# BluemlJ/oc_cleanrl

Measured on AMD Instinct MI355X. Metric: env steps/sec (SPS) + PPO updates/sec, ALE/Pong-v5 obj-mode, 1/2/4/8 MI355X, higher is better.
Workload: dtype fp32

## Files before the change

### include/ocppo.h

```cpp
#ifndef OCPPO_H
#define OCPPO_H

#include <stddef.h>
#include <stdint.h>

#ifdef __cplusplus
extern "C" {
#endif

#define OCPPO_ABI_VERSION 30

#define OCPPO_OK 0
#define OCPPO_E_INVALID 1
#define OCPPO_E_LAUNCH 2
#define OCPPO_E_WORKSPACE 3

#define OCPPO_F32 0
#define OCPPO_BF16 1
#define OCPPO_U8 2

#define OCPPO_NET_CHANNELS_LAST 1
#define OCPPO_NET_SCALE_255 2

#define OCPPO_STAT_LOSS 0
#define OCPPO_STAT_PG_LOSS 1
#define OCPPO_STAT_V_LOSS 2
#define OCPPO_STAT_ENTROPY 3
#define OCPPO_STAT_OLD_APPROX_KL 4
#define OCPPO_STAT_APPROX_KL 5
#define OCPPO_STAT_CLIPFRAC 6
#define OCPPO_STAT_ADV_MEAN 7
#define OCPPO_STAT_ADV_STD 8
#define OCPPO_NUM_STATS 9

typedef void* ocppo_stream_t;
typedef struct ocppo_deferred_finish {
  uint64_t opaque[64];
} ocppo_deferred_finish_t;

#if defined(__GNUC__) || defined(__clang__)
#define OCPPO_API __attribute__((visibility("default")))
#else
#define OCPPO_API
// ... 361 lines not shown
                                    int norm_adv, int clip_vloss, float* gp, float* db_h,
                                    float* dwa, float* dwc, float* dba, float* dbc, float* stats,
                                    float* dlogits, float* dvalue, void* workspace,
                                    size_t workspace_bytes, ocppo_deferred_finish_t* finish);
OCPPO_API int ocppo_sum_splits_finish(ocppo_stream_t stream, const float* part, int64_t S,
                                      int64_t n, float* out, const ocppo_deferred_finish_t* finish);
OCPPO_API int ocppo_deferred_finish_run(ocppo_stream_t stream,
                                        const ocppo_deferred_finish_t* finish);

OCPPO_API int ocppo_linear_cache_shift(ocppo_stream_t stream, const float* x, int64_t ldx,
                                       const float* w, const float* b, float* enc,
                                       const float* done, int64_t M, int64_t N, int64_t K,
                                       int64_t W, int relu);
OCPPO_API int ocppo_linear_cache_ring(ocppo_stream_t stream, const float* x, int64_t ldx,
                                      const float* w, const float* b, float* enc,
                                      const float* done, int64_t M, int64_t N, int64_t K,
                                      int64_t W, int64_t slot, int relu);
OCPPO_API int ocppo_linear_act_ring(ocppo_stream_t stream, const float* x, int64_t ldx,
                                    const float* w, const float* b, float* y, int64_t ldy,
                                    int64_t M, int64_t N, int64_t K, int64_t seg, int64_t rot,
                                    int relu);
OCPPO_API int ocppo_conv2d_act(ocppo_stream_t stream, const float* x, int64_t B, int64_t H,
                               int64_t W, int64_t Cin, const float* w, const float* b,
                               int64_t Cout, int64_t KH, int64_t KW, int64_t stride, float* y,
                               int relu);
OCPPO_API int ocppo_store_linear2(ocppo_stream_t stream, const float* frame, const float* reward,
                                  const float* done, int64_t N, int64_t W, int64_t D,
                                  const void* prev_obs, void* obs_out, int obs_dtype,
                                  float* net_obs, float* reward_out, float* done_out, int vecnorm,
                                  double gamma, double epsilon, double clip_reward,
                                  double* ret_state, double* rms_state, const float* w1,
                                  const float* b1, const float* w2, const float* b2, float* y,
                                  int64_t ldy, int64_t N1, int64_t N2);

OCPPO_API int ocppo_cartpole_step(ocppo_stream_t stream, uint64_t seed, const int64_t* actions,
                                  int64_t N, double* state, int64_t* counters, float* obs_out,
                                  float* reward_out, float* done_out, float* ep_state);

#ifdef __cplusplus
}
#endif
#endif
```

### oc_cleanrl_amd/_lib.py

```python
from __future__ import annotations

import ctypes
import os
import re
from pathlib import Path

import torch

PKG = Path(__file__).resolve().parent
LIB_PATH = Path(os.environ.get("OCPPO_LIB", PKG / "lib" / "libocppo_hip.so"))
HEADER = PKG.parent / "include" / "ocppo.h"

OCPPO_ABI_VERSION = 30
OCPPO_OK, OCPPO_E_INVALID, OCPPO_E_LAUNCH, OCPPO_E_WORKSPACE = 0, 1, 2, 3
OCPPO_F32, OCPPO_BF16, OCPPO_U8 = 0, 1, 2
OCPPO_X6_MBITS_ROWS = 2
STAT_NAMES = ("loss", "pg_loss", "v_loss", "entropy", "old_approx_kl", "approx_kl", "clipfrac",
              "adv_mean", "adv_std")
OCPPO_NUM_STATS = len(STAT_NAMES)

P, I64, U64, D, I, SZ = (ctypes.c_void_p, ctypes.c_int64, ctypes.c_uint64, ctypes.c_double,
                         ctypes.c_int, ctypes.c_size_t)

SIGNATURES: dict[str, tuple[type, list]] = {
    "ocppo_abi_version": (I, []),
    "ocppo_last_error": (ctypes.c_char_p, []),
    "ocppo_gae": (I, [P, P, P, P, P, P, I64, I64, D, D, P, P]),
    "ocppo_minibatch_adv_stats": (I, [P, P, P, I64, I64, P]),
    "ocppo_minibatch_prepare": (I, [P, P, I64, I64, P, P, P, P, P, P, P, P, P, P, P]),
    "ocppo_ppo_loss_workspace_bytes": (SZ, [I64, I64]),
    "ocppo_ppo_loss_fwd_bwd": (I, [P, P, P, I64, I64, P, P, P, P, P, P, P, D, D, D, I, I, P, P, P,
                                   P, SZ]),
    "ocppo_clip_adam_workspace_bytes": (SZ, [I64]),
    "ocppo_clip_adam_step": (I, [P, P, P, P, P, I64, P, D, D, D, D, D, P, P, SZ, I, P, P, P, P,
                                 P]),
    "ocppo_categorical_sample": (I, [P, P, P, P, I64, I64, I64, I64, P, P, P, P, P]),
    "ocppo_policy_head_sample": (I, [P, P, I64, I64, P, P, P, P, P, P, I64, I64, I64, P, P, P, P,
                                     P]),
    "ocppo_torch_exponential_geometry": (I, [I64, I64, I64, P, P]),
    "ocppo_philox_exponential": (I, [P, P, I64, P, I64, I64]),
    "ocppo_philox_exponential_steps": (I, [P, P, I64, I64, P, I64, I64, I64]),
    "ocppo_categorical_logprob_entropy": (I, [P, P, P, I64, I64, P, P]),
    "ocppo_categorical_logprob_entropy_bwd": (I, [P, P, P, P, P, I64, I64, P]),
    "ocppo_rollout_store": (I, [P, P, I, P, P, I64, I64, I64, P, P, I, P, P, P, I, P]),
    "ocppo_obs_reset": (I, [P, P, I, I64, I64, I64, P, I, P, I]),
    "ocppo_gather_rows": (I, [P, P, I, P, I64, I64, P]),
# ... 51 lines not shown
    "ocppo_sum_splits_finish": (I, [P, P, I64, I64, P, P]),
    "ocppo_sum_splits_act": (I, [P, P, I64, I64, I64, P, I, P]),
    "ocppo_gemm_x6_gather": (I, [P, P, I64, I64, P, I64, I64, P, I64, I64, I64, I64, I64, I64, P,
                                 I, P, P, I64, I64, I]),
    "ocppo_frames_expand_index": (I, [P, P, P, I64, P, I64, I64, I64, P]),
    "ocppo_gemm_x6_wgrad": (I, [P, P, I64, I64, P, I64, I64, I64, I64, I64, P, I64, P, I64, I64,
                                P, P, P, I64, I, P]),
    "ocppo_conv_x6": (I, [P, I, P, P, P, I64, P, I64, I64, I64, I64, I64, P, I, P, I, P, P, P,
                          P, P, P]),
    "ocppo_conv_x6_u8": (I, [P, I, P, P, I64, I64, I64, I64, I64, I64, P, I64, P, I64, I64, I64,
                             I64, P, I, ctypes.c_float, I, P, P, P, P]),
    "ocppo_deferred_finish_run": (I, [P, P]),
    "ocppo_linear_cache_shift": (I, [P, P, I64, P, P, P, P, I64, I64, I64, I64, I]),
    "ocppo_linear_cache_ring": (I, [P, P, I64, P, P, P, P, I64, I64, I64, I64, I64, I]),
    "ocppo_linear_act_ring": (I, [P, P, I64, P, P, P, I64, I64, I64, I64, I64, I64, I]),
    "ocppo_conv2d_act": (I, [P, P, I64, I64, I64, I64, P, P, I64, I64, I64, I64, P, I]),
    "ocppo_frames_scatter_chunks": (I64, [I64]),
    "ocppo_frames_gather_linear": (I, [P, P, I, I64, I64, I64, I64, P, I64, P, P, I64, I, P, P, P,
                                       P, I64, P, P]),
    "ocppo_q_head_epsilon_greedy": (I, [P, P, I64, I64, P, P, I64, U64, P, I64, D, D, D, P, P, P]),
    "ocppo_dqn_act_step": (I, [P, P, I64, I64, P, P, I64, U64, P, I64, D, D, D, P, P, U64, P, I64,
                               I64, P, P, P, P, I64, P, P, I, P, P, P, I, D, D, D, P, P, P, I64, P,
                               P, P, P, I64]),
    "ocppo_frames_scatter_relu": (I, [P, P, I64, I64, P, I64, P, I64, P, I64, I64, I64, P, P, P,
                                      P]),
    "ocppo_gemm_x6": (I, [P, P, I64, I64, P, I64, I64, P, I64, I64, I64, I64, I64, I64, P, I, P,
                          I64, P, P, P, I, I, P, I64, I64, P, SZ]),
    "ocppo_gemm_x6_sk_workspace_bytes": (SZ, [I]),
    "ocppo_split_planes": (I, [P, I, P, P, P, P, P, P]),
    "ocppo_gae_records": (I, [P, P, P, P, P, P, I64, I64, D, D, P, P, P, P, P]),
    "ocppo_minibatch_prepare_records": (I, [P, P, I64, I64, P, P, P, P, P, P, P]),
    "ocppo_store_linear2": (I, [P, P, P, P, I64, I64, I64, P, P, I, P, P, P, I, D, D, D, P, P, P,
                                P, P, P, P, I64, I64, I64]),
}


class OcppoError(RuntimeError):
    """A C-ABI call returned a non-zero status."""


def header_functions() -> list[str]:
    text = HEADER.read_text()
    return sorted(set(re.findall(r"^\s*(?:const\s+)?[\w\s\*]*?\b(ocppo_\w+)\s*\(", text, re.M)))


def _load() -> ctypes.CDLL:
    if not LIB_PATH.exists():
        raise ImportError(
            f"{LIB_PATH} is missing: the HIP extension is required (no CPU fallback). "
            "Build it with `python -m oc_cleanrl_amd.build`.")
    lib = ctypes.CDLL(str(LIB_PATH))
    for name, (restype, argtypes) in SIGNATURES.items():
        fn = getattr(lib, name)
        fn.restype = restype
        fn.argtypes = argtypes
    ver = lib.ocppo_abi_version()
    if ver != OCPPO_ABI_VERSION:
        raise ImportError(f"{LIB_PATH}: ABI version {ver}, expected {OCPPO_ABI_VERSION}; rebuild")
    return lib


LIB = _load()


def call(name: str, *args) -> None:
    rc = getattr(LIB, name)(*args)
# ... 4 lines not shown
```

### oc_cleanrl_amd/csrc/ocppo_linear.hip

```cpp
#include "ocppo_common.h"

namespace ocppo {

typedef float floatx4 __attribute__((ext_vector_type(4)));

#ifndef OCPPO_LIN_MAX_WAVES
#define OCPPO_LIN_MAX_WAVES 8
#endif
#ifndef OCPPO_LIN_WAVE_TARGET
#define OCPPO_LIN_WAVE_TARGET 4096
#endif
constexpr int kLinMaxWaves = OCPPO_LIN_MAX_WAVES;

template <int CH, bool VEC>
__device__ __forceinline__ void linear_wave_chunks(const float* xr, const float* wr, bool rok,
                                                   bool cok, int K, int g, int c0, int c1,
                                                   floatx4& acc0, floatx4& acc1) {
  for (int cb = c0; cb < c1; cb += CH) {
    float4 a[CH], bb[CH];
#pragma unroll
    for (int q = 0; q < CH; ++q) {
      const int k = (cb + q) * 16 + 4 * g;
      const bool live = cb + q < c1;
      if (VEC && k + 3 < K) {
// ... 498 lines not shown
                                       const float* w, const float* b, float* enc,
                                       const float* done, int64_t M, int64_t N, int64_t K,
                                       int64_t W, int64_t slot, int relu) {
  OCPPO_REQUIRE(M >= 0 && N >= 1 && K >= 1 && W >= 1 && W <= 64 && M <= INT32_MAX &&
                    N <= INT32_MAX && K <= INT32_MAX && slot >= 0 && slot < W,
                "ocppo_linear_cache_ring: bad sizes M=%lld N=%lld K=%lld W=%lld slot=%lld",
                (long long)M, (long long)N, (long long)K, (long long)W, (long long)slot);
  OCPPO_REQUIRE(ldx >= K, "ocppo_linear_cache_ring: ldx=%lld < K", (long long)ldx);
  if (M == 0) return OCPPO_OK;
  OCPPO_REQUIRE(x && w && enc, "ocppo_linear_cache_ring: null pointer");
  OCPPO_REQUIRE((M + 15) / 16 * ((N + 15) / 16) <= INT32_MAX / 8,
                "ocppo_linear_cache_ring: too large");
  const bool vec = K % 4 == 0 && ldx % 4 == 0 && reinterpret_cast<uintptr_t>(x) % 16 == 0 &&
                   reinterpret_cast<uintptr_t>(w) % 16 == 0;
  const CacheOut c{enc, done, static_cast<int>(W), static_cast<int>(slot)};
  clear_stale_error();
  hipStream_t s = as_stream(stream);
  if (relu)
    launch_linear<true, true>(s, vec, x, ldx, w, b, nullptr, 0, (int)M, (int)N, (int)K, c);
  else
    launch_linear<false, true>(s, vec, x, ldx, w, b, nullptr, 0, (int)M, (int)N, (int)K, c);
  return check_launch("ocppo_linear_cache_ring");
}

namespace ocppo {

constexpr int kLin2MaxK1 = 64;
constexpr int kLin2MaxN1 = 512;

template <int S, bool RELU1, bool RELU2, int XDT>
__device__ __forceinline__ void linear2_tile(
    int b, float* smem, const float* __restrict__ x, int64_t ldx, const float* __restrict__ w1,
    const float* __restrict__ b1, const float* __restrict__ w2, const float* __restrict__ b2,
    float* __restrict__ y, int64_t ldy, int M, int N1, int N2, int K1, int ntm, int tiles) {
  const int ldh = N1 + 4;
  float* h1 = smem;
  floatx4* red = reinterpret_cast<floatx4*>(smem + 16 * ldh);
  const int per_xcd = (tiles + 7) / 8;
  const int t = (b % 8) * per_xcd + b / 8;
  if (t >= tiles) return;
  const int tm = t % ntm, tn = t / ntm;
  const int lane = threadIdx.x & 63, wv = threadIdx.x >> 6;
  const int g = lane >> 4, c16 = lane & 15;
  const int row = tm * 16 + c16;
  const bool rok = row < M;
  const float* xr = x + static_cast<int64_t>(rok ? row : 0) * ldx;

  const int nkc = (K1 + 15) / 16;
  const int nct = N1 / 16;
  const int col2 = tn * 16 + c16;
  const bool cok = col2 < N2;
  const float* w2r = w2 + static_cast<int64_t>(cok ? col2 : 0) * N1;
  const int cpw = (nct + S - 1) / S;
  const int c0 = wv * cpw;
  const int c1 = c0 + cpw < nct ? c0 + cpw : nct;
  constexpr int kMaxT = kLin2MaxN1 / 16 / S;
  float4 a1[kLin2MaxK1 / 16];
#pragma unroll
  for (int kc = 0; kc < kLin2MaxK1 / 16; ++kc) {
    const int k = kc * 16 + 4 * g;
    a1[kc].x = (kc < nkc && rok && k + 0 < K1) ? Elem<XDT>::roundtrip(xr[k + 0]) : 0.f;
    a1[kc].y = (kc < nkc && rok && k + 1 < K1) ? Elem<XDT>::roundtrip(xr[k + 1]) : 0.f;
    a1[kc].z = (kc < nkc && rok && k + 2 < K1) ? Elem<XDT>::roundtrip(xr[k + 2]) : 0.f;
    a1[kc].w = (kc < nkc && rok && k + 3 < K1) ? Elem<XDT>::roundtrip(xr[k + 3]) : 0.f;
  }
  float4 b2v[kMaxT];
#pragma unroll
  for (int q = 0; q < kMaxT; ++q) {
    const int c = c0 + q;
    b2v[q] = (c < c1 && cok) ? *reinterpret_cast<const float4*>(w2r + c * 16 + 4 * g)
                             : make_float4(0.f, 0.f, 0.f, 0.f);
  }
#pragma unroll
  for (int q = 0; q < kMaxT; ++q) {
    const int ct = wv + q * S;
    if (ct < nct) {
      const int col = ct * 16 + c16;
      const float* wr = w1 + static_cast<int64_t>(col) * K1;
      floatx4 acc = {0.f, 0.f, 0.f, 0.f};
// ... 185 lines not shown
                "ocppo_store_linear2: bad sizes N=%lld W=%lld D=%lld N1=%lld N2=%lld (D <= 64, "
                "N1 %% 16 == 0, N1 <= 512)", (long long)N, (long long)W, (long long)D,
                (long long)N1, (long long)N2);
  OCPPO_REQUIRE(obs_dtype == OCPPO_F32 || obs_dtype == OCPPO_BF16,
                "ocppo_store_linear2: obs dtype must be OCPPO_F32 or OCPPO_BF16 (object vectors)");
  OCPPO_REQUIRE(frame && reward && done && prev_obs && obs_out && w1 && w2 && y,
                "ocppo_store_linear2: null pointer");
  OCPPO_REQUIRE(prev_obs != obs_out, "ocppo_store_linear2: prev_obs must not alias obs_out");
  OCPPO_REQUIRE(!vecnorm || (ret_state && rms_state && reward_out && reward_out != reward),
                "ocppo_store_linear2: VecNormalize needs ret/rms state and a separate reward_out");
  OCPPO_REQUIRE(reinterpret_cast<uintptr_t>(w2) % 16 == 0,
                "ocppo_store_linear2: w2 must be 16-B aligned");
  StoreLin2Args a;
  a.frame = frame; a.reward = reward; a.done = done; a.N = N; a.D = D; a.W = (int)W;
  a.prev = prev_obs; a.out = obs_out; a.net = net_obs; a.reward_out = reward_out;
  a.done_out = done_out; a.gamma = gamma; a.eps = epsilon; a.clip = clip_reward;
  a.ret = ret_state; a.rms = rms_state;
  a.w1 = w1; a.b1 = b1; a.w2 = w2; a.b2 = b2; a.y = y; a.ldy = ldy;
  a.N1 = (int)N1; a.N2 = (int)N2;
  a.ntm = (int)((N + 15) / 16);
  a.tiles = a.ntm * (int)((N2 + 15) / 16);
  a.lin_blocks = 8 * ((a.tiles + 7) / 8);
  clear_stale_error();
  hipStream_t s = as_stream(stream);
  if (obs_dtype == OCPPO_BF16) {
    if (vecnorm) launch_store_linear2<OCPPO_BF16, true>(s, a);
    else launch_store_linear2<OCPPO_BF16, false>(s, a);
  } else {
    if (vecnorm) launch_store_linear2<OCPPO_F32, true>(s, a);
    else launch_store_linear2<OCPPO_F32, false>(s, a);
  }
  return check_launch("ocppo_store_linear2");
}
```

### oc_cleanrl_amd/csrc/ocppo_synth_env.h

```cpp
#pragma once
#include "ocppo_common.h"

namespace ocppo {

__device__ __forceinline__ uint64_t splitmix64(uint64_t x) {
  x += 0x9E3779B97F4A7C15ull;
  x = (x ^ (x >> 30)) * 0xBF58476D1CE4E5B9ull;
  x = (x ^ (x >> 27)) * 0x94D049BB133111EBull;
  return x ^ (x >> 31);
}
__device__ __forceinline__ float unit24(uint64_t h) {
  return static_cast<float>(h >> 40) * (1.0f / 16777216.0f);
}

__device__ __forceinline__ uint64_t synth_env_key(uint64_t seed, uint64_t step, int64_t n) {
  return splitmix64(splitmix64(splitmix64(seed) + step) + static_cast<uint64_t>(n));
}

__device__ __forceinline__ uint32_t synth_env_obj_base(uint64_t key, int64_t k) {
  const uint64_t h = splitmix64(key + static_cast<uint64_t>(k));
  const int field = static_cast<int>(k & 3);
  if (field == 0) return static_cast<uint32_t>(h % 160u);
  if (field == 1) return static_cast<uint32_t>(h % 210u);
  return static_cast<uint32_t>(1u + h % 16u);
}
__device__ __forceinline__ float synth_env_obj_act(uint32_t base, int64_t k, int64_t a) {
  const uint64_t v = (k == 1) ? (base + 7u * static_cast<uint64_t>(a)) % 210u : base;
  return static_cast<float>(v);
}
__device__ __forceinline__ float synth_env_obj(uint64_t key, int64_t k, int64_t a) {
  return synth_env_obj_act(synth_env_obj_base(key, k), k, a);
}

__device__ __forceinline__ uint8_t synth_env_pixel(uint64_t key, int64_t k, int64_t a) {
  const uint64_t h = splitmix64(key + static_cast<uint64_t>(k));
  uint32_t v = (h % 10u == 0u) ? static_cast<uint32_t>((h >> 8) & 0xFFu) : 0u;
  if (k < 84) v = static_cast<uint32_t>((a * 37) & 0xFF);
  return static_cast<uint8_t>(v);
}

__device__ __forceinline__ void synth_env_outcome(uint64_t key, int64_t n,
                                                  float* __restrict__ reward_out,
                                                  float* __restrict__ done_out,
                                                  float* __restrict__ ep) {
  const float ur = unit24(splitmix64(key ^ 0x5DEECE66Dull));
  const float r = ur < 0.005f ? 1.f : (ur < 0.01f ? -1.f : 0.f);
  const float ud = unit24(splitmix64(key ^ 0xB5297A4Dull));
  const float d = ud < (1.0f / 3500.0f) ? 1.f : 0.f;
  reward_out[n] = r;
  done_out[n] = d;
  if (ep) {
    float* e = ep + n * 5;
    const float run_ret = e[0] + r, run_len = e[1] + 1.f;
    if (d != 0.f) {
      e[2] += run_ret;
      e[3] += run_len;
      e[4] += 1.f;
      e[0] = 0.f;
      e[1] = 0.f;
    } else {
      e[0] = run_ret;
      e[1] = run_len;
    }
  }
}

}
```

### oc_cleanrl_amd/ops.py

```python
from __future__ import annotations

import ctypes

import torch

from . import _lib
from ._lib import OCPPO_BF16, OCPPO_F32, OCPPO_U8, STAT_NAMES, call

_DTYPE_CODE = {torch.float32: OCPPO_F32, torch.bfloat16: OCPPO_BF16, torch.uint8: OCPPO_U8}


def _check(t: torch.Tensor, name: str, dtype: torch.dtype | None = None, device=None,
           numel: int | None = None) -> int:
    if not isinstance(t, torch.Tensor):
        raise TypeError(f"{name}: expected a tensor, got {type(t).__name__}")
    if t.device.type != "cuda":
        raise ValueError(f"{name}: HIP kernels need a GPU tensor, got device {t.device}")
    if device is not None and t.device != device:
        raise ValueError(f"{name}: on {t.device}, expected {device}")
    if dtype is not None and t.dtype != dtype:
        raise ValueError(f"{name}: dtype {t.dtype}, expected {dtype}")
    if not t.is_contiguous():
        raise ValueError(f"{name}: must be contiguous")
    if numel is not None and t.numel() != numel:
# ... 1062 lines not shown


def store_linear2(frame, reward, done, prev_obs, obs_out, net_obs, done_out, reward_out, w1, b1,
                  w2, b2, y, vecnorm_state=None, gamma=0.99, epsilon=1e-8, clip_reward=10.0):
    N, D = frame.shape
    W = obs_out.shape[1]
    dev = frame.device
    f = torch.float32
    if frame.dtype != f:
        raise ValueError("store_linear2: object frames only (f32)")
    if prev_obs.shape != obs_out.shape or prev_obs.dtype != obs_out.dtype or \
            tuple(obs_out.shape) != (N, W, D) or obs_out.dtype not in (torch.float32, torch.bfloat16):
        raise ValueError(f"obs slots must be [N, W, D] f32|bf16, got {tuple(obs_out.shape)} "
                         f"{obs_out.dtype}")
    N1, N2 = w1.shape[0], w2.shape[0]
    if tuple(w1.shape) != (N1, D) or tuple(w2.shape) != (N2, N1) or y.shape[0] != N or \
            y.shape[1] != N2 or y.stride(1) != 1 or y.dtype != f:
        raise ValueError(f"shapes: frame {tuple(frame.shape)}, w1 {tuple(w1.shape)}, "
                         f"w2 {tuple(w2.shape)}, y {tuple(y.shape)}")
    vn = vecnorm_state is not None
    ret, rms = vecnorm_state if vn else (None, None)
    call("ocppo_store_linear2", _stream(dev), _check(frame, "frame", f, dev),
         _check(reward, "reward", f, dev, N), _check(done, "done", f, dev, N), N, W, D,
         _check(prev_obs, "prev_obs", None, dev), _check(obs_out, "obs_out", None, dev),
         _DTYPE_CODE[obs_out.dtype], _opt(net_obs, "net_obs", f, dev, N * W * D),
         _check(reward_out, "reward_out", f, dev, N), _opt(done_out, "done_out", f, dev, N),
         int(vn), float(gamma), float(epsilon), float(clip_reward),
         _opt(ret, "ret_state", torch.float64, dev, N), _opt(rms, "rms_state", torch.float64, dev, 3),
         _check(w1, "w1", f, dev), _opt(b1, "b1", f, dev, N1), _check(w2, "w2", f, dev),
         _opt(b2, "b2", f, dev, N2), y.data_ptr(), y.stride(0) if N > 1 else N2, N1, N2)
    return y


_RB_WS: dict = {}


def _relu_bias_ws(R: int, N: int, dev):
    key = (dev, R, N)
    ws = _RB_WS.get(key)
    if ws is None:
        nb = int(_lib.LIB.ocppo_relu_bias_grad_workspace_bytes(R, N))
        ws = _RB_WS[key] = torch.zeros(nb, dtype=torch.uint8, device=dev)
    return ws


def relu_bias_grad_ok(g) -> bool:
    return (g.is_cuda and g.dtype == torch.float32 and g.dim() == 2 and g.shape[1] % 4 == 0
            and 4 <= g.shape[1] <= 16384 and g.is_contiguous() and g.data_ptr() % 16 == 0)


def relu_bias_grad(g, out=None, db=None, gp=None, bits=None):
    if g.dim() != 2:
        raise ValueError(f"g must be [R, N], got {tuple(g.shape)}")
    R, N = g.shape
    dev = g.device
    f = torch.float32
    if db is None:
        db = torch.empty(N, dtype=f, device=dev)
    if bits is not None:
        gp = torch.empty_like(g) if gp is None else gp
        ws = _relu_bias_ws(R, N, dev)
        call("ocppo_relu_bias_grad_bits", _stream(dev), _check(g, "g", f, dev),
             _check(bits, "bits", torch.int32, dev, R * N // 32), _check(gp, "gp", f, dev, R * N),
             _check(db, "db", f, dev, N), R, N, ws.data_ptr(), ws.numel())
        return gp, db
    if out is not None and gp is None:
# ... 1158 lines not shown
```

### oc_cleanrl_amd/trainer.py

```python
from __future__ import annotations

import json
import math
import os
import time
from dataclasses import asdict
from pathlib import Path

import numpy as np
import torch
import torch.distributed as dist
import torch.nn as nn

from . import agents, frames, gemm_table, ops, rccl
from .rccl import RcclComm, RcclExchange
from .agents import NormalizeImg, PPObj, fused_trunk, linear_relu, make_agent
from .args import Args
from .envs import HostVecEnv, make_device_env


def storage_dtype(args: Args, pixels: bool, integer_obs: bool = True) -> torch.dtype:
    choice = args.obs_storage
    if choice == "auto":
        if pixels:
            return torch.uint8
        return torch.bfloat16 if args.noise_std == 0.0 and integer_obs else torch.float32
    return {"f32": torch.float32, "bf16": torch.bfloat16, "u8": torch.uint8}[choice]


FUSED_HEAD_ENV = True
ADAM_WRITES_PLANES = False
FUSED_HEADS_LOSS_ANY_TRUNK = True
STAGE_ON_SIDE_STREAM = False
U8_ROLLOUT_CONV = True


class FlatGrads:

    def __init__(self, params):
        self.params = [p for p in params if p.requires_grad]
        offs, n = ops.flat_offsets(self.params)
        dev = self.params[0].device
        self.buf = torch.zeros(n, dtype=torch.float32, device=dev)
        for p, off in zip(self.params, offs):
            p.grad = self.buf[off:off + p.numel()].as_strided(p.shape, p.stride())
        self.numel = n

    def zero(self):
        self.buf.zero_()

    def allreduce_mean(self, group=None):
        ws = dist.get_world_size(group)
        dist.all_reduce(self.buf, op=dist.ReduceOp.SUM, group=group)
        self.buf.div_(ws)


class GradExchange:

    def __init__(self, buf, tail_off: int, world: int, scale_in_optimizer: bool, group=None):
        self.buf, self.tail_off, self.world = buf, tail_off, world
        self.scale_in_optimizer, self.group = scale_in_optimizer, group

    def _finish(self):
# ... 190 lines not shown
            self.lr = self.optimizer.lr
        else:
            grads = FlatGrads(self.agent.parameters())
            self.params = grads.params
            self.grad_buf = grads.buf
            self.lr = torch.tensor(a.learning_rate, dtype=torch.float32, device=self.dev)
            self.optimizer = torch.optim.Adam(self.params, lr=self.lr, eps=1e-5, fused=True,
                                              capturable=True)

        T, N = self.T, self.N
        f32 = torch.float32
        dev = self.dev
        self.obs_dtype = storage_dtype(a, self.pixels, not self.host_env and
                                       getattr(self.env, "integer_obs", False))
        self.obs = torch.zeros((T + 1, N) + self.obs_shape, dtype=self.obs_dtype, device=dev)
        self.net_obs = torch.empty((N,) + self.obs_shape, dtype=f32, device=dev,
                                   memory_format=self.net_format).zero_()
        self.actions = torch.zeros((T, N), dtype=torch.int64, device=dev)
        self.logprobs = torch.zeros((T, N), dtype=f32, device=dev)
        self.rewards = torch.zeros((T, N), dtype=f32, device=dev)
        self.dones = torch.zeros((T + 1, N), dtype=f32, device=dev)
        self.values = torch.zeros((T + 1, N), dtype=f32, device=dev)
        self.advantages = torch.zeros((T, N), dtype=f32, device=dev)
        self.returns = torch.zeros((T, N), dtype=f32, device=dev)
        self.noise = torch.zeros((T, N, self.A), dtype=f32, device=dev)
        self.exp_stream = (ops.TorchExpStream(N * self.A, dev)
                           if a.sampling_noise in ("kernel", "head") else None)
        self.enc_cache = (torch.zeros((N, self.obs_shape[0], self.agent.encoding_dim), dtype=f32,
                                      device=dev) if self.frame_cache else None)
        self.rollout_fusion = self.frame_cache and a.rollout_fusion and self._fusable_encoder()
        self.enc_pair = (torch.zeros((N, self.agent.network[2].out_features), dtype=f32, device=dev)
                         if self.rollout_fusion else None)
        self.cache_ring = self.rollout_fusion and a.rollout_cache_ring and self._ring_decoder()
        self.ret_state = torch.zeros(N, dtype=torch.float64, device=dev)
        self.rms_state = torch.tensor([0.0, 1.0, 1e-4], dtype=torch.float64, device=dev)

        self.B = a.local_batch_size
        self.M = a.local_minibatch_size
        self.E = a.update_epochs
        self.nmb = a.num_minibatches
        self.b_inds = np.arange(self.B)
        self.perm_host = torch.empty(self.E * self.B, dtype=torch.int64, pin_memory=True)
        self.perm_dev = torch.zeros(self.E * self.B, dtype=torch.int64, device=dev)
        self.perm_stage = torch.zeros_like(self.perm_dev)
        self.staged = False
        self.staged_rng_state = self.current_rng_state = None
        self.executed_mb = self.E * self.nmb
        self._pending_metrics, self._metrics_host, self._metrics_turn = None, [None, None], 0
        self.perm_event = torch.cuda.Event()
        self.perm_event.record()
        self.copy_stream = (torch.cuda.Stream(dev) if STAGE_ON_SIDE_STREAM and
                            torch.device(dev).type == "cuda" else None)
        self.stage_read = torch.cuda.Event()
        W = self.obs_shape[0]
        self.frame_dedup = (a.update_frame_dedup and isinstance(self.agent, PPObj) and
                            not self.reset_stacks and
                            not self.pixels and len(self.obs_shape) == 2 and
                            len(a.encoder_dims) > 0 and 1 <= W <= 16)
        self.planner = (frames.FramePlanner(T, N, W, a.local_minibatch_size, a.update_epochs,
                                            a.num_minibatches) if self.frame_dedup else None)
        self.plan_host = self.plan_stage = self.plan_dev = self.plan = None
        self.split, self.tail_off, self.cuts = 0, 0, {}
        if self.dp and a.dp_overlap and self.frame_dedup and len(a.encoder_dims) >= 2:
            self.split = 2 * (len(a.encoder_dims) - 1)
            first_tail = self.agent.network[self.split].weight
            offs, _ = ops.flat_offsets(self.params)
# ... 125 lines not shown
        if not self.cache_ring:
            return self.enc_cache
        return torch.roll(self.enc_cache, -(t % self.enc_cache.shape[1]), dims=1)

    def _reset_env(self):
        frame = self.env.frame if self.host_env else self.env.reset()
        if self.reset_stacks:
            ones = torch.ones(self.N, dtype=torch.float32, device=self.dev)
            ops.rollout_store(frame, ones, ones, self.obs[0], self.obs[self.T], self._store_net,
                              scale255=self.prescale, reset_prev=self.env.reset_prev)
        else:
            ops.obs_reset(frame, self.obs[self.T], self._store_net, scale255=self.prescale)
        self.dones[self.T].zero_()

    def _policy_hidden(self, t: int):
        if not self.frame_cache:
            if self.u8_rollout:
                return self.agent.trunk_frames(self.obs[t], self.env_rows)
            return self.agent.trunk(self.net_obs, self.prescale)
        self._policy_encode(t)
        return self._decode_cache(t)

    def _policy_encode(self, t: int):
        ag = self.agent
        if t == 0:
            self.enc_cache.copy_(ag.encode(self.net_obs))
        elif self.rollout_fusion:
            self._store_encode(t)
        else:
            fresh = ag.encode(self.net_obs[:, -1])
            self.timer.bracket("frame_cache", lambda: ops.frame_cache_shift(
                self.enc_cache, fresh, self.dones[t]))

    def _store_encode(self, t: int):
        a, env, net = self.args, self.env, self.agent.network
        lins = [m for m in net[:self.agent._flat] if isinstance(m, nn.Linear)]
        vn = (self.ret_state, self.rms_state) if a.vecnorm_reward else None
        self.timer.bracket("store_encode", lambda: ops.store_linear2(
            env.frame, env.reward, env.done, self.obs[t - 1], self.obs[t], self.net_obs,
            self.dones[t], self.rewards[t - 1], lins[0].weight, lins[0].bias, lins[1].weight,
            lins[1].bias, self.enc_pair, vecnorm_state=vn))
        x = self.enc_pair
        for i, lin in enumerate(lins[2:-1]):
            x = self.timer.bracket("encoder_mid" if i == 0 else f"encoder_mid{i}",
                                   lambda x=x, lin=lin: linear_relu(x, lin))
        last = lins[-1]
        if self.cache_ring:
            W = self.enc_cache.shape[1]
            self.timer.bracket("cache_linear", lambda: ops.linear_cache_ring(
                x, last.weight, last.bias, self.enc_cache, (t - 1) % W, self.dones[t]))
        else:
            self.timer.bracket("cache_linear", lambda: ops.linear_cache_shift(
                x, last.weight, last.bias, self.enc_cache, self.dones[t]))

    def _rollout_step(self, t: int):
        if not self._act(t, env_step=True):
            self.timer.bracket("env_step", lambda: self.env.step(self.actions[t], t))
        if not self.rollout_fusion:
            self._store(t)

    def _act(self, t: int, env_step: bool = False) -> bool:
        ag = self.agent
        if self.args.sampling_noise == "torch":
            self.noise[t].exponential_()
        px = self.exp_stream.philox(t) if self.args.sampling_noise == "head" else None
        if self.fused_head:
            hidden = self._policy_hidden(t)
            if env_step and FUSED_HEAD_ENV and ops.policy_head_env_ok(
                    hidden, ag.actor.weight, ag.critic.weight, self.env):
                self.timer.bracket("action_head_env", lambda: ops.policy_head_env_step(
                    hidden, ag.actor.weight, ag.actor.bias, ag.critic.weight, ag.critic.bias,
                    self.noise[t], self.actions[t], self.logprobs[t], self.values[t], self.env,
                    t, philox=px))
                return True
            self.timer.bracket("action_head", lambda: ops.policy_head_sample(
                hidden, ag.actor.weight, ag.actor.bias, ag.critic.weight, ag.critic.bias,
                self.noise[t], self.actions[t], self.logprobs[t], self.values[t], philox=px))
        else:
            logits, value = (ag.heads(ag.trunk_frames(self.obs[t], self.env_rows))
                             if self.u8_rollout else ag.logits_and_value(self.net_obs, self.prescale))
            self.timer.bracket("action_head", lambda: ops.categorical_sample(
                logits, self.noise[t], self.actions[t], self.logprobs[t], None, value.view(-1),
                self.values[t], philox=px))
        return False

    def _store(self, t: int):
        a = self.args
        rp = self.env.reset_prev if self.reset_stacks else None
        if a.vecnorm_reward:
            self.timer.bracket("rollout_store", lambda: ops.rollout_store_vecnorm(
                self.env.frame, self.env.reward, self.env.done, self.obs[t], self.obs[t + 1],
                self._store_net, self.dones[t + 1], self.ret_state, self.rms_state, self.rewards[t],
                scale255=self.prescale, reset_prev=rp))
        else:
            self.timer.bracket("rollout_store", lambda: ops.rollout_store(
                self.env.frame, self.env.reward, self.env.done, self.obs[t], self.obs[t + 1],
                self._store_net, self.rewards[t], self.dones[t + 1], scale255=self.prescale,
                reset_prev=rp))

    def _rollout_begin(self):
# ... 4 lines not shown
            self.noise.exponential_()
        elif self.args.sampling_noise == "kernel":
            self.timer.bracket("noise_draws", lambda: self.exp_stream.fill(self.noise))

    def _rollout_end(self):
        a = self.args
        T = self.T
        if self.frame_cache:
            self.values[T].copy_(self.agent._head(self.agent.critic,
                                                  self._policy_hidden(T)).view(-1))
        elif self.u8_rollout:
            self.values[T].copy_(self.agent._head(
                self.agent.critic, self.agent.trunk_frames(self.obs[T], self.env_rows)).view(-1))
        else:
            self.values[T].copy_(self.agent.get_value(self.net_obs, self.prescale).view(-1))
        rec = self.records
        self.timer.bracket("gae", lambda: ops.gae(
            self.rewards, self.values[:T], self.dones[:T], self.values[T], self.dones[T],
            a.gamma, a.gae_lambda, self.advantages, self.returns, logprobs=self.logprobs,
            actions=self.actions, records=rec))
        self._prepare_minibatches(from_records=rec is not None)

    def _prepare_minibatches(self, from_records: bool = False):
        T = self.T
        rec = self.records if from_records else None
        self.timer.bracket("mb_prepare", lambda: ops.minibatch_prepare(
            self.perm_dev, self.M, self.actions.view(-1), self.logprobs.view(-1),
            self.advantages.view(-1), self.returns.view(-1), self.values[:T].reshape(-1),
            out=self.mb, with_stats=self.args.norm_adv, records=rec))

    def _rollout(self):
        with torch.no_grad(), agents.rollout_inference():
            self._rollout_begin()
            for t in range(self.T):
                self._rollout_step(t)
            self.env.advance(self.T)
            self._rollout_end()

    def _host_part(self, k: int):
        with torch.no_grad():
            if k == 0:
                self._rollout_begin()
            else:
                self.env.upload()
                if not self.rollout_fusion:
                    self._store(k - 1)
            if k < self.T:
                self._act(k)
                self.env.fetch_actions(self.actions[k])
            else:
                self._rollout_end()

    def _rollout_host(self):
        for k in range(self.T + 1):
            if k > 0:
                self.env.upload_resets()
            if self.g_host:
                self.g_host[k].replay()
            else:
                self._host_part(k)
            if k < self.T:
                self.env.host_step()

    def _forward_backward(self, j: int):
        if not self.wplanes_built:
            self.wplanes, self.wplanes_built = self._weight_planes(), True
            self.planes_by_opt = (ADAM_WRITES_PLANES and self.wplanes is not None
                                  and self.args.fused_optimizer and len(self.wplanes.jobs) <= 8
# ... 471 lines not shown
```

Measured before the change: 1.024 million.

## Fuse policy head, synthetic env step and store+encoder into one rollout kernel

Adds a kernel that, per 16-row tile, computes the policy head sampling, generates the synthetic env frame/reward/done, writes the observation window and runs the first two encoder linears from LDS. The rollout loop uses it to merge the action-head-env launch with the store_linear2 launch for each step, so there are fewer kernel launches per env step and the frame no longer round-trips through global memory. Linear tile blocks recompute the head and env rows redundantly, and a separate block recomputes rewards for vecnorm, adding some extra compute and register pressure.

After: 1.042 million, median of 6. 1.8% higher.

```diff
diff --git a/include/ocppo.h b/include/ocppo.h
--- a/include/ocppo.h
+++ b/include/ocppo.h
@@ -8,7 +8,7 @@
 extern "C" {
 #endif
 
-#define OCPPO_ABI_VERSION 30
+#define OCPPO_ABI_VERSION 31
 
 #define OCPPO_OK 0
 #define OCPPO_E_INVALID 1
@@ -436,6 +436,16 @@
                                   double* ret_state, double* rms_state, const float* w1,
                                   const float* b1, const float* w2, const float* b2, float* y,
                                   int64_t ldy, int64_t N1, int64_t N2);
+OCPPO_API int ocppo_head_env_store_linear2(
+    ocppo_stream_t stream, const float* hidden, int64_t H, const float* w_actor,
+    const float* b_actor, const float* w_critic, const float* b_critic, const float* noise,
+    int64_t A, int64_t* action_out, float* logprob_out, float* value_out, uint64_t seed,
+    const int64_t* step_base, int64_t step_offset, float* frame_out, float* env_reward_out,
+    float* env_done_out, float* ep_state, int64_t N, int64_t W, int64_t D, const void* prev_obs,
+    void* obs_out, int obs_dtype, float* net_obs, float* reward_out, float* done_out, int vecnorm,
+    double gamma, double epsilon, double clip_reward, double* ret_state, double* rms_state,
+    const float* w1, const float* b1, const float* w2, const float* b2, float* y, int64_t ldy,
+    int64_t N1, int64_t N2);
 
 OCPPO_API int ocppo_cartpole_step(ocppo_stream_t stream, uint64_t seed, const int64_t* actions,
                                   int64_t N, double* state, int64_t* counters, float* obs_out,
diff --git a/oc_cleanrl_amd/_lib.py b/oc_cleanrl_amd/_lib.py
--- a/oc_cleanrl_amd/_lib.py
+++ b/oc_cleanrl_amd/_lib.py
@@ -11,7 +11,7 @@
 LIB_PATH = Path(os.environ.get("OCPPO_LIB", PKG / "lib" / "libocppo_hip.so"))
 HEADER = PKG.parent / "include" / "ocppo.h"
 
-OCPPO_ABI_VERSION = 30
+OCPPO_ABI_VERSION = 31
 OCPPO_OK, OCPPO_E_INVALID, OCPPO_E_LAUNCH, OCPPO_E_WORKSPACE = 0, 1, 2, 3
 OCPPO_F32, OCPPO_BF16, OCPPO_U8 = 0, 1, 2
 OCPPO_X6_MBITS_ROWS = 2
@@ -129,6 +129,9 @@
     "ocppo_minibatch_prepare_records": (I, [P, P, I64, I64, P, P, P, P, P, P, P]),
     "ocppo_store_linear2": (I, [P, P, P, P, I64, I64, I64, P, P, I, P, P, P, I, D, D, D, P, P, P,
                                 P, P, P, P, I64, I64, I64]),
+    "ocppo_head_env_store_linear2": (I, [P, P, I64, P, P, P, P, P, I64, P, P, P, U64, P, I64, P, P,
+                                         P, P, I64, I64, I64, P, P, I, P, P, P, I, D, D, D, P, P,
+                                         P, P, P, P, P, I64, I64, I64]),
 }
 
 
diff --git a/oc_cleanrl_amd/csrc/ocppo_linear.hip b/oc_cleanrl_amd/csrc/ocppo_linear.hip
--- a/oc_cleanrl_amd/csrc/ocppo_linear.hip
+++ b/oc_cleanrl_amd/csrc/ocppo_linear.hip
@@ -554,7 +554,8 @@
 __device__ __forceinline__ void linear2_tile(
     int b, float* smem, const float* __restrict__ x, int64_t ldx, const float* __restrict__ w1,
     const float* __restrict__ b1, const float* __restrict__ w2, const float* __restrict__ b2,
-    float* __restrict__ y, int64_t ldy, int M, int N1, int N2, int K1, int ntm, int tiles) {
+    float* __restrict__ y, int64_t ldy, int M, int N1, int N2, int K1, int ntm, int tiles,
+    int xrow0 = 0) {
   const int ldh = N1 + 4;
   float* h1 = smem;
   floatx4* red = reinterpret_cast<floatx4*>(smem + 16 * ldh);
@@ -566,7 +567,7 @@
   const int g = lane >> 4, c16 = lane & 15;
   const int row = tm * 16 + c16;
   const bool rok = row < M;
-  const float* xr = x + static_cast<int64_t>(rok ? row : 0) * ldx;
+  const float* xr = x + static_cast<int64_t>(rok ? row - xrow0 : 0) * ldx;
 
   const int nkc = (K1 + 15) / 16;
   const int nct = N1 / 16;
@@ -818,3 +819,248 @@
   }
   return check_launch("ocppo_store_linear2");
 }
+
+#include "ocppo_categorical.h"
+#include "ocppo_synth_env.h"
+
+namespace ocppo {
+
+struct HeadEnvArgs {
+  const float* hidden;
+  const float* wa;
+  const float* ba;
+  const float* wc;
+  const float* bc;
+  const float* noise;
+  int A;
+  int64_t* action_out;
+  float* logprob_out;
+  float* value_out;
+  uint64_t seed;
+  const int64_t* step_base;
+  int64_t step_offset;
+  float* frame;
+  float* reward;
+  float* done;
+  float* ep;
+};
+
+struct HeadEnvRows {
+  float frame[16 * kLin2MaxK1];
+  float logit[16][9];
+  float reward[16];
+  float done[16];
+};
+
+template <int CH>
+__device__ __forceinline__ void head_env_rows(const HeadEnvArgs& h, int row0, int N, int D,
+                                              bool owner, HeadEnvRows& s) {
+  const int tid = threadIdx.x, lane = tid & (kWave - 1), wv = tid / kWave;
+  const int A = h.A;
+  const int jo = lane >> 3;
+  const float bias = jo < A ? h.ba[jo] : (jo == 7 ? h.bc[0] : 0.f);
+  float4 w[8][CH];
+#pragma unroll
+  for (int j = 0; j < 8; ++j) {
+    const float* wrow = j == 7 ? h.wc : h.wa + j * (256 * CH);
+#pragma unroll
+    for (int c = 0; c < CH; ++c)
+      w[j][c] = (j < A || j == 7) ? reinterpret_cast<const float4*>(wrow)[c * kWave + lane]
+                                  : make_float4(0.f, 0.f, 0.f, 0.f);
+  }
+  float4 x[4][CH];
+#pragma unroll
+  for (int q = 0; q < 4; ++q) {
+    const int row = row0 + 4 * wv + q;
+    if (row < N) {
+      head_load_row<CH>(h.hidden, row, lane, x[q]);
+    } else {
+#pragma unroll
+      for (int c = 0; c < CH; ++c) x[q][c] = make_float4(0.f, 0.f, 0.f, 0.f);
+    }
+  }
+  const int64_t trow = row0 + lane;
+  const bool tl = wv == 0 && lane < 16 && trow < N;
+  float nzj[7];
+#pragma unroll
+  for (int j = 0; j < 7; ++j) nzj[j] = (tl && j < A) ? h.noise[trow * A + j] : 1.f;
+  const uint64_t step = static_cast<uint64_t>(h.step_base[0] + h.step_offset);
+  for (int e = tid; e < 16 * D; e += blockDim.x) {
+    const int r = e / D, k = e - r * D;
+    if (row0 + r < N && k != 1)
+      s.frame[e] = synth_env_obj(synth_env_key(h.seed, step, row0 + r), k, 0);
+  }
+#pragma unroll
+  for (int q = 0; q < 4; ++q) {
+    const float t = head_dots<CH>(x[q], w, lane) + bias;
+    if ((lane & 7) == 0) s.logit[4 * wv + q][jo] = t;
+  }
+  __syncthreads();
+  if (tl) {
+    float l[8];
+#pragma unroll
+    for (int j = 0; j < 8; ++j) l[j] = s.logit[lane][j];
+    const uint64_t key = synth_env_key(h.seed, step, trow);
+    const int best = head_tail(l, nzj, A, trow, h.action_out, h.logprob_out, nullptr, h.value_out,
+                               nullptr, owner);
+    if (D > 1) s.frame[lane * D + 1] = synth_env_obj(key, 1, best);
+    float r, d;
+    synth_env_reward_done(key, r, d);
+    s.reward[lane] = r;
+    s.done[lane] = d;
+    if (owner) synth_env_outcome(key, trow, h.reward, h.done, h.ep);
+  }
+  __syncthreads();
+  if (owner) {
+    for (int e = tid; e < 16 * D; e += blockDim.x)
+      if (row0 + e / D < N) h.frame[static_cast<int64_t>(row0) * D + e] = s.frame[e];
+  }
+}
+
+template <int ODT, int VEC>
+__device__ __forceinline__ void store_rows_lds(const HeadEnvRows& s, int row0, int nrows, int W,
+                                               int D, const void* __restrict__ prev,
+                                               void* __restrict__ out, float* __restrict__ net,
+                                               float* __restrict__ reward_out,
+                                               float* __restrict__ done_out) {
+  const int DG = D / VEC;
+  const int groups = nrows * W * DG;
+  for (int g = threadIdx.x; g < groups; g += blockDim.x) {
+    const int r = g / (W * DG);
+    const int rem = g - r * W * DG;
+    const int w = rem / DG;
+    const int k = (rem - w * DG) * VEC;
+    const int64_t n = row0 + r;
+    float v[VEC];
+    if (w == W - 1 || s.done[r] != 0.f) {
+#pragma unroll
+      for (int q = 0; q < VEC; ++q) v[q] = s.frame[r * D + k + q];
+    } else {
+      VecIO<ODT, VEC>::load(prev, (n * W + w + 1) * D + k, v);
+    }
+    const int64_t o = (n * W + w) * D + k;
+    VecIO<ODT, VEC>::store(out, o, v);
+    if (net) {
+      float back[VEC];
+#pragma unroll
+      for (int q = 0; q < VEC; ++q) back[q] = Elem<ODT>::roundtrip(v[q]);
+      VecIO<OCPPO_F32, VEC>::store(net, o, back);
+    }
+  }
+  if (static_cast<int>(threadIdx.x) < nrows) {
+    const int64_t n = row0 + threadIdx.x;
+    if (reward_out) reward_out[n] = s.reward[threadIdx.x];
+    if (done_out) done_out[n] = s.done[threadIdx.x];
+  }
+}
+
+template <int ODT, int VEC, bool VN, int CH>
+__global__ __launch_bounds__(256) void head_env_store_linear2_kernel(HeadEnvArgs h,
+                                                                     StoreLin2Args a) {
+  extern __shared__ __attribute__((aligned(16))) float smem[];
+  __shared__ HeadEnvRows rows;
+  const int b = blockIdx.x;
+  const int N = static_cast<int>(a.N), D = static_cast<int>(a.D);
+  if (b < a.lin_blocks) {
+    const int per_xcd = (a.tiles + 7) / 8;
+    const int t = (b % 8) * per_xcd + b / 8;
+    if (t >= a.tiles) return;
+    const int tm = t % a.ntm;
+    head_env_rows<CH>(h, tm * 16, N, D, false, rows);
+    linear2_tile<4, true, true, ODT>(b, smem, rows.frame, a.D, a.w1, a.b1, a.w2, a.b2, a.y, a.ldy,
+                                     N, a.N1, a.N2, D, a.ntm, a.tiles, tm * 16);
+    return;
+  }
+  if (VN && b == a.lin_blocks) {
+    const uint64_t step = static_cast<uint64_t>(h.step_base[0] + h.step_offset);
+    for (int n = threadIdx.x; n < N; n += blockDim.x)
+      synth_env_reward_done(synth_env_key(h.seed, step, n), smem[n], smem[N + n]);
+    __syncthreads();
+    vecnorm_block(smem, smem + N, a.N, a.gamma, a.eps, a.clip, a.ret, a.rms, a.reward_out);
+    return;
+  }
+  const int row0 = (b - a.lin_blocks - (VN ? 1 : 0)) * 16;
+  head_env_rows<CH>(h, row0, N, D, true, rows);
+  store_rows_lds<ODT, VEC>(rows, row0, N - row0 < 16 ? N - row0 : 16, a.W, D, a.prev, a.out, a.net,
+                           VN ? nullptr : a.reward_out, a.done_out);
+}
+
+template <int ODT, bool VN, int CH>
+static void launch_head_env_store_linear2(hipStream_t s, const HeadEnvArgs& h,
+                                          const StoreLin2Args& a) {
+  size_t lds = sizeof(float) * 16 * (a.N1 + 4) + sizeof(floatx4) * 64 * 3;
+  if (VN && lds < sizeof(float) * 2 * a.N) lds = sizeof(float) * 2 * a.N;
+  const dim3 grid(a.lin_blocks + (VN ? 1 : 0) + a.ntm);
+  if (a.D % 4 == 0)
+    hipLaunchKernelGGL((head_env_store_linear2_kernel<ODT, 4, VN, CH>), grid, dim3(256), lds, s, h,
+                       a);
+  else
+    hipLaunchKernelGGL((head_env_store_linear2_kernel<ODT, 1, VN, CH>), grid, dim3(256), lds, s, h,
+                       a);
+}
+
+template <int CH>
+static void launch_head_env_store_linear2_dt(hipStream_t s, int obs_dtype, bool vn,
+                                             const HeadEnvArgs& h, const StoreLin2Args& a) {
+  if (obs_dtype == OCPPO_BF16) {
+    if (vn) launch_head_env_store_linear2<OCPPO_BF16, true, CH>(s, h, a);
+    else launch_head_env_store_linear2<OCPPO_BF16, false, CH>(s, h, a);
+  } else {
+    if (vn) launch_head_env_store_linear2<OCPPO_F32, true, CH>(s, h, a);
+    else launch_head_env_store_linear2<OCPPO_F32, false, CH>(s, h, a);
+  }
+}
+
+}
+
+extern "C" int ocppo_head_env_store_linear2(
+    ocppo_stream_t stream, const float* hidden, int64_t H, const float* w_actor,
+    const float* b_actor, const float* w_critic, const float* b_critic, const float* noise,
+    int64_t A, int64_t* action_out, float* logprob_out, float* value_out, uint64_t seed,
+    const int64_t* step_base, int64_t step_offset, float* frame_out, float* env_reward_out,
+    float* env_done_out, float* ep_state, int64_t N, int64_t W, int64_t D, const void* prev_obs,
+    void* obs_out, int obs_dtype, float* net_obs, float* reward_out, float* done_out, int vecnorm,
+    double gamma, double epsilon, double clip_reward, double* ret_state, double* rms_state,
+    const float* w1, const float* b1, const float* w2, const float* b2, float* y, int64_t ldy,
+    int64_t N1, int64_t N2) {
+  const char* const fn = "ocppo_head_env_store_linear2";
+  OCPPO_REQUIRE(N >= 1 && N <= 4096 && W >= 1 && W <= 64 && D >= 1 && D <= kLin2MaxK1 &&
+                    N1 >= 16 && N1 % 16 == 0 && N1 <= kLin2MaxN1 && N2 >= 1 && N2 <= INT32_MAX &&
+                    ldy >= N2 && (H == 256 || H == 512) && A >= 1 && A <= 7,
+                "%s: bad sizes N=%lld W=%lld D=%lld N1=%lld N2=%lld H=%lld A=%lld (N <= 4096, "
+                "D <= 64, N1 %% 16 == 0, N1 <= 512, H 256 or 512, A <= 7)", fn, (long long)N,
+                (long long)W, (long long)D, (long long)N1, (long long)N2, (long long)H,
+                (long long)A);
+  OCPPO_REQUIRE(obs_dtype == OCPPO_F32 || obs_dtype == OCPPO_BF16,
+                "%s: obs dtype must be OCPPO_F32 or OCPPO_BF16 (object vectors)", fn);
+  OCPPO_REQUIRE(hidden && w_actor && b_actor && w_critic && b_critic && noise && action_out &&
+                    logprob_out && value_out && step_base && frame_out && env_reward_out &&
+                    env_done_out && prev_obs && obs_out && reward_out && w1 && w2 && y,
+                "%s: null pointer", fn);
+  OCPPO_REQUIRE(prev_obs != obs_out, "%s: prev_obs must not alias obs_out", fn);
+  OCPPO_REQUIRE(!vecnorm || (ret_state && rms_state && reward_out != env_reward_out),
+                "%s: VecNormalize needs ret/rms state and a separate reward_out", fn);
+  OCPPO_REQUIRE(((reinterpret_cast<uintptr_t>(hidden) | reinterpret_cast<uintptr_t>(w_actor) |
+                  reinterpret_cast<uintptr_t>(w_critic) | reinterpret_cast<uintptr_t>(w2)) & 15) == 0,
+                "%s: hidden, head weights and w2 must be 16-B aligned", fn);
+  HeadEnvArgs h;
+  h.hidden = hidden; h.wa = w_actor; h.ba = b_actor; h.wc = w_critic; h.bc = b_critic;
+  h.noise = noise; h.A = (int)A; h.action_out = action_out; h.logprob_out = logprob_out;
+  h.value_out = value_out; h.seed = seed; h.step_base = step_base; h.step_offset = step_offset;
+  h.frame = frame_out; h.reward = env_reward_out; h.done = env_done_out; h.ep = ep_state;
+  StoreLin2Args a;
+  a.frame = nullptr; a.reward = nullptr; a.done = nullptr; a.N = N; a.D = D; a.W = (int)W;
+  a.prev = prev_obs; a.out = obs_out; a.net = net_obs; a.reward_out = reward_out;
+  a.done_out = done_out; a.gamma = gamma; a.eps = epsilon; a.clip = clip_reward;
+  a.ret = ret_state; a.rms = rms_state;
+  a.w1 = w1; a.b1 = b1; a.w2 = w2; a.b2 = b2; a.y = y; a.ldy = ldy;
+  a.N1 = (int)N1; a.N2 = (int)N2;
+  a.ntm = (int)((N + 15) / 16);
+  a.tiles = a.ntm * (int)((N2 + 15) / 16);
+  a.lin_blocks = 8 * ((a.tiles + 7) / 8);
+  clear_stale_error();
+  hipStream_t s = as_stream(stream);
+  if (H == 256) launch_head_env_store_linear2_dt<1>(s, obs_dtype, vecnorm != 0, h, a);
+  else launch_head_env_store_linear2_dt<2>(s, obs_dtype, vecnorm != 0, h, a);
+  return check_launch(fn);
+}
diff --git a/oc_cleanrl_amd/csrc/ocppo_synth_env.h b/oc_cleanrl_amd/csrc/ocppo_synth_env.h
--- a/oc_cleanrl_amd/csrc/ocppo_synth_env.h
+++ b/oc_cleanrl_amd/csrc/ocppo_synth_env.h
@@ -39,14 +39,19 @@
   return static_cast<uint8_t>(v);
 }
 
+__device__ __forceinline__ void synth_env_reward_done(uint64_t key, float& r, float& d) {
+  const float ur = unit24(splitmix64(key ^ 0x5DEECE66Dull));
+  r = ur < 0.005f ? 1.f : (ur < 0.01f ? -1.f : 0.f);
+  const float ud = unit24(splitmix64(key ^ 0xB5297A4Dull));
+  d = ud < (1.0f / 3500.0f) ? 1.f : 0.f;
+}
+
 __device__ __forceinline__ void synth_env_outcome(uint64_t key, int64_t n,
                                                   float* __restrict__ reward_out,
                                                   float* __restrict__ done_out,
                                                   float* __restrict__ ep) {
-  const float ur = unit24(splitmix64(key ^ 0x5DEECE66Dull));
-  const float r = ur < 0.005f ? 1.f : (ur < 0.01f ? -1.f : 0.f);
-  const float ud = unit24(splitmix64(key ^ 0xB5297A4Dull));
-  const float d = ud < (1.0f / 3500.0f) ? 1.f : 0.f;
+  float r, d;
+  synth_env_reward_done(key, r, d);
   reward_out[n] = r;
   done_out[n] = d;
   if (ep) {
diff --git a/oc_cleanrl_amd/ops.py b/oc_cleanrl_amd/ops.py
--- a/oc_cleanrl_amd/ops.py
+++ b/oc_cleanrl_amd/ops.py
@@ -1118,6 +1118,54 @@
     return y
 
 
+def head_env_store_linear2_ok(hidden, w_actor, w_critic, env) -> bool:
+    return policy_head_env_ok(hidden, w_actor, w_critic, env) and hidden.shape[1] in (256, 512) \
+        and env.frame.shape[1] <= 64
+
+
+def head_env_store_linear2(hidden, w_actor, b_actor, w_critic, b_critic, noise, action_out,
+                           logprob_out, value_out, env, step_offset: int, prev_obs, obs_out,
+                           net_obs, done_out, reward_out, w1, b1, w2, b2, y, vecnorm_state=None,
+                           gamma=0.99, epsilon=1e-8, clip_reward=10.0):
+    N, H = hidden.shape
+    A = w_actor.shape[0]
+    D = env.frame.shape[1]
+    W = obs_out.shape[1]
+    dev = hidden.device
+    f = torch.float32
+    if tuple(w_actor.shape) != (A, H) or w_critic.numel() != H or b_actor.numel() != A:
+        raise ValueError("head weights do not match hidden")
+    if prev_obs.shape != obs_out.shape or prev_obs.dtype != obs_out.dtype or \
+            tuple(obs_out.shape) != (N, W, D) or obs_out.dtype not in (torch.float32, torch.bfloat16):
+        raise ValueError(f"obs slots must be [N, W, D] f32|bf16, got {tuple(obs_out.shape)} "
+                         f"{obs_out.dtype}")
+    N1, N2 = w1.shape[0], w2.shape[0]
+    if tuple(w1.shape) != (N1, D) or tuple(w2.shape) != (N2, N1) or y.shape[0] != N or \
+            y.shape[1] != N2 or y.stride(1) != 1 or y.dtype != f:
+        raise ValueError(f"shapes: frame {tuple(env.frame.shape)}, w1 {tuple(w1.shape)}, "
+                         f"w2 {tuple(w2.shape)}, y {tuple(y.shape)}")
+    vn = vecnorm_state is not None
+    ret, rms = vecnorm_state if vn else (None, None)
+    call("ocppo_head_env_store_linear2", _stream(dev), _check(hidden, "hidden", f, dev), H,
+         _check(w_actor, "w_actor", f, dev), _check(b_actor, "b_actor", f, dev, A),
+         _check(w_critic, "w_critic", f, dev, H), _check(b_critic, "b_critic", f, dev, 1),
+         _check(noise, "noise", f, dev, N * A), A,
+         _check(action_out, "action_out", torch.int64, dev, N),
+         _check(logprob_out, "logprob_out", f, dev, N), _check(value_out, "value_out", f, dev, N),
+         env.seed & 0xFFFFFFFFFFFFFFFF, _check(env.step_base, "step_base", torch.int64, dev, 1),
+         int(step_offset), _check(env.frame, "frame", f, dev, N * D),
+         _check(env.reward, "reward", f, dev, N), _check(env.done, "done", f, dev, N),
+         _opt(env.ep_state, "ep_state", f, dev, N * 5), N, W, D,
+         _check(prev_obs, "prev_obs", None, dev), _check(obs_out, "obs_out", None, dev),
+         _DTYPE_CODE[obs_out.dtype], _opt(net_obs, "net_obs", f, dev, N * W * D),
+         _check(reward_out, "reward_out", f, dev, N), _opt(done_out, "done_out", f, dev, N),
+         int(vn), float(gamma), float(epsilon), float(clip_reward),
+         _opt(ret, "ret_state", torch.float64, dev, N), _opt(rms, "rms_state", torch.float64, dev, 3),
+         _check(w1, "w1", f, dev), _opt(b1, "b1", f, dev, N1), _check(w2, "w2", f, dev),
+         _opt(b2, "b2", f, dev, N2), y.data_ptr(), y.stride(0) if N > 1 else N2, N1, N2)
+    return y
+
+
 _RB_WS: dict = {}
 
 
diff --git a/oc_cleanrl_amd/trainer.py b/oc_cleanrl_amd/trainer.py
--- a/oc_cleanrl_amd/trainer.py
+++ b/oc_cleanrl_amd/trainer.py
@@ -29,6 +29,7 @@
 
 
 FUSED_HEAD_ENV = True
+ROLLOUT_FUSED_STEP = True
 ADAM_WRITES_PLANES = False
 FUSED_HEADS_LOSS_ANY_TRUNK = True
 STAGE_ON_SIDE_STREAM = False
@@ -285,6 +286,11 @@
         self.enc_pair = (torch.zeros((N, self.agent.network[2].out_features), dtype=f32, device=dev)
                          if self.rollout_fusion else None)
         self.cache_ring = self.rollout_fusion and a.rollout_cache_ring and self._ring_decoder()
+        self.fused_step_ok = (
+            self.rollout_fusion and not self.host_env and T >= 2 and
+            a.sampling_noise in ("kernel", "rollout") and ops.head_env_store_linear2_ok(
+                torch.empty((N, self.H), dtype=f32, device=dev), self.agent.actor.weight,
+                self.agent.critic.weight, self.env))
         self.ret_state = torch.zeros(N, dtype=torch.float64, device=dev)
         self.rms_state = torch.tensor([0.0, 1.0, 1e-4], dtype=torch.float64, device=dev)
 
@@ -476,14 +482,23 @@
             self.timer.bracket("frame_cache", lambda: ops.frame_cache_shift(
                 self.enc_cache, fresh, self.dones[t]))
 
-    def _store_encode(self, t: int):
+    def _store_encode(self, t: int, hidden=None):
         a, env, net = self.args, self.env, self.agent.network
+        ag = self.agent
         lins = [m for m in net[:self.agent._flat] if isinstance(m, nn.Linear)]
         vn = (self.ret_state, self.rms_state) if a.vecnorm_reward else None
-        self.timer.bracket("store_encode", lambda: ops.store_linear2(
-            env.frame, env.reward, env.done, self.obs[t - 1], self.obs[t], self.net_obs,
-            self.dones[t], self.rewards[t - 1], lins[0].weight, lins[0].bias, lins[1].weight,
-            lins[1].bias, self.enc_pair, vecnorm_state=vn))
+        if hidden is not None:
+            self.timer.bracket("head_store_encode", lambda: ops.head_env_store_linear2(
+                hidden, ag.actor.weight, ag.actor.bias, ag.critic.weight, ag.critic.bias,
+                self.noise[t - 1], self.actions[t - 1], self.logprobs[t - 1], self.values[t - 1],
+                env, t - 1, self.obs[t - 1], self.obs[t], self.net_obs, self.dones[t],
+                self.rewards[t - 1], lins[0].weight, lins[0].bias, lins[1].weight, lins[1].bias,
+                self.enc_pair, vecnorm_state=vn))
+        else:
+            self.timer.bracket("store_encode", lambda: ops.store_linear2(
+                env.frame, env.reward, env.done, self.obs[t - 1], self.obs[t], self.net_obs,
+                self.dones[t], self.rewards[t - 1], lins[0].weight, lins[0].bias, lins[1].weight,
+                lins[1].bias, self.enc_pair, vecnorm_state=vn))
         x = self.enc_pair
         for i, lin in enumerate(lins[2:-1]):
             x = self.timer.bracket("encoder_mid" if i == 0 else f"encoder_mid{i}",
@@ -503,13 +518,14 @@
         if not self.rollout_fusion:
             self._store(t)
 
-    def _act(self, t: int, env_step: bool = False) -> bool:
+    def _act(self, t: int, env_step: bool = False, hidden=None) -> bool:
         ag = self.agent
         if self.args.sampling_noise == "torch":
             self.noise[t].exponential_()
         px = self.exp_stream.philox(t) if self.args.sampling_noise == "head" else None
         if self.fused_head:
-            hidden = self._policy_hidden(t)
+            if hidden is None:
+                hidden = self._policy_hidden(t)
             if env_step and FUSED_HEAD_ENV and ops.policy_head_env_ok(
                     hidden, ag.actor.weight, ag.critic.weight, self.env):
                 self.timer.bracket("action_head_env", lambda: ops.policy_head_env_step(
@@ -580,8 +596,16 @@
     def _rollout(self):
         with torch.no_grad(), agents.rollout_inference():
             self._rollout_begin()
-            for t in range(self.T):
-                self._rollout_step(t)
+            if self.fused_step_ok and ROLLOUT_FUSED_STEP and FUSED_HEAD_ENV:
+                hidden = self._policy_hidden(0)
+                for t in range(1, self.T):
+                    self._store_encode(t, hidden)
+                    hidden = self._decode_cache(t)
+                ran = self._act(self.T - 1, env_step=True, hidden=hidden)
+                assert ran
+            else:
+                for t in range(self.T):
+                    self._rollout_step(t)
             self.env.advance(self.T)
             self._rollout_end()
 
```
